# iaomw/Tracer

Measured on AMD Instinct MI355X. Metric: Mrays/s at 1920x1080x64spp, higher is better.
Workload: dtype f32

## Files before the change

### tracer_amd/csrc/dev_intersect.hpp

```cpp
#pragma once

#include "dev_prof.hpp"
#include "dev_scene.hpp"
#include "dev_vec.hpp"

namespace trcdev {

constexpr int kBlock = 64;

struct Ray {
    F3 o, d, inv;
};
TRC_DEV Ray make_ray(F3 o, F3 dir) {
    Ray r; r.o = o; r.d = normalize(dir); r.inv = rcp_cr(r.d); return r;
}
TRC_DEV F3 point_at(const Ray& r, float t) { return r.o + r.d * t; }

struct HitRec {
    float t;
    F3 p, gn, sn;
    F2 uv;
    uint32_t material;
    float PDF;
    uint32_t tag;
    F3 vol_o, vol_d;
    float vol_t;
    uint32_t vol_cube;
};
TRC_DEV void hit_init(HitRec& h) {
    h.t = 0; h.p = f3(0); h.gn = f3(0); h.sn = f3(0); h.uv.x = 0; h.uv.y = 0; h.material = 0; h.PDF = 0; h.tag = kTagNone;
    h.vol_o = f3(0); h.vol_d = f3(0); h.vol_t = 0; h.vol_cube = kTagNone;
}
TRC_DEV void check_face(HitRec& h, const Ray& ray) {
    bool f = dot(ray.d, h.gn) <= 0;
    h.sn = f ? h.gn : -h.gn;
}

struct SceneRef {
    const uint32_t* small_base;
    const uint32_t* blob;
    uint32_t off_nodes, off_spheres, off_squares, off_cubes, off_materials, off_tripos, off_triattr;
    uint32_t n_lds_nodes;
    uint32_t stack_lds;
    uint32_t stack_cap;
    uint32_t* ovf;
    uint32_t descend_min;
};
TRC_DEV float4 ld4(const uint32_t* p) { return *reinterpret_cast<const float4*>(p); }
#if defined(__HIP_DEVICE_COMPILE__)
typedef float trc_v4f __attribute__((ext_vector_type(4)));
TRC_DEV float4 ld4_global(const uint32_t* p) {
    const trc_v4f v = *(const __attribute__((address_space(1))) trc_v4f*)p;
    return make_float4(v.x, v.y, v.z, v.w);
}
TRC_DEV float4 ld4_lds(const uint32_t* p) {
    const trc_v4f v = *(const __attribute__((address_space(3))) trc_v4f*)p;
    return make_float4(v.x, v.y, v.z, v.w);
}
TRC_DEV uint32_t ld1_global(const uint32_t* p) { return *(const __attribute__((address_space(1))) uint32_t*)p; }
TRC_DEV void st1_global(uint32_t* p, uint32_t v) { *(__attribute__((address_space(1))) uint32_t*)p = v; }
#else
TRC_DEV float4 ld4_global(const uint32_t* p) { return ld4(p); }
TRC_DEV float4 ld4_lds(const uint32_t* p) { return ld4(p); }
TRC_DEV uint32_t ld1_global(const uint32_t* p) { return *p; }
TRC_DEV void st1_global(uint32_t* p, uint32_t v) { *p = v; }
#endif

template <bool ALL_LDS>
TRC_DEV void load_node(const SceneRef& S, uint32_t idx, float4& q0, float4& q1, float4& q2, float4& q3) {
    if (ALL_LDS || idx < S.n_lds_nodes) {
        const uint32_t* np = S.small_base + S.off_nodes + idx * kNodeDwords;
        q0 = ld4_lds(np); q1 = ld4_lds(np + 4); q2 = ld4_lds(np + 8); q3 = ld4_lds(np + 12);
    } else {
        const uint32_t* np = S.blob + S.off_nodes + (size_t)idx * kNodeDwords;
        q0 = ld4_global(np); q1 = ld4_global(np + 4); q2 = ld4_global(np + 8); q3 = ld4_global(np + 12);
    }
}

#ifndef TRC_WALK_TRIM
#define TRC_WALK_TRIM 1
#endif
constexpr float kRangeTMin = FLT_MIN;
static_assert(!TRC_WALK_TRIM || kRangeTMin > 0, "box_hit / box_hit_t drop `|| tmax < 0` and `tmin < 0 ? tmax : tmin`: valid for a positive lower bound only");
TRC_DEV bool box_hit(F3 mn, F3 mx, const Ray& r, float ry) {
    F3 ts = (mn - r.o) * r.inv;
    F3 te = (mx - r.o) * r.inv;
    float tmin = fmax3(fminf(ts.x, te.x), fminf(ts.y, te.y), fminf(ts.z, te.z));
    float tmax = fmin3(fmaxf(ts.x, te.x), fmaxf(ts.y, te.y), fmaxf(ts.z, te.z));
    tmin = fmaxf(tmin, kRangeTMin);
    tmax = fminf(tmax, ry);
    return !(tmax < tmin || (!TRC_WALK_TRIM && tmax < 0));
}
TRC_DEV bool box_hit_t(F3 mn, F3 mx, const Ray& r, float ry, float& t) {
    F3 ts = (mn - r.o) * r.inv;
    F3 te = (mx - r.o) * r.inv;
    float tmin = fmax3(fminf(ts.x, te.x), fminf(ts.y, te.y), fminf(ts.z, te.z));
    float tmax = fmin3(fmaxf(ts.x, te.x), fmaxf(ts.y, te.y), fmaxf(ts.z, te.z));
    tmin = fmaxf(tmin, kRangeTMin);
    tmax = fminf(tmax, ry);
    if (tmax < tmin || (!TRC_WALK_TRIM && tmax < 0)) return false;
    t = (!TRC_WALK_TRIM && tmin < 0) ? tmax : tmin;
    return true;
}

TRC_DEV float box_pad() { return 1 + 2 * ((3 * FLT_EPSILON * 0.5f) / (1 - 3 * FLT_EPSILON * 0.5f)); }

TRC_DEV bool box_hit_record(F3 mini, F3 maxi, F3 o, F3 d, float range_y, float& out_t, F3& out_gn, F3& out_p, F2& out_uv) {
    float tmin = -FLT_MAX;
    float tmax = range_y;
    uint32_t axisPick = 0;
    const F3 ddd = o - mini, bbb = o - maxi;
    const float pad = box_pad();
    const bool inside = (ddd.x > 0 && ddd.y > 0 && ddd.z > 0) && (bbb.x < 0 && bbb.y < 0 && bbb.z < 0);
#if TRC_WAVE_GUARDS
    const F3 nlo = mini - o, nhi = maxi - o;
    F3 qlo, qhi;
    {
        const GuardedDivBy bx = guarded_div_by(d.x), by = guarded_div_by(d.y), bz = guarded_div_by(d.z);
        qlo = f3(div_core(nlo.x, bx), div_core(nlo.y, by), div_core(nlo.z, bz));
        qhi = f3(div_core(nhi.x, bx), div_core(nhi.y, by), div_core(nhi.z, bz));
        const float small = fminf(fmin3(fmin3(fabsf(nlo.x), fabsf(nlo.y), fabsf(nlo.z)), fmin3(fabsf(nhi.x), fabsf(nhi.y), fabsf(nhi.z)),
                                        fmin3(fabsf(d.x), fabsf(d.y), fabsf(d.z))), 0x1p60f);
        const float large = fmax3(fmax3(fabsf(nlo.x), fabsf(nlo.y), fabsf(nlo.z)), fmax3(fabsf(nhi.x), fabsf(nhi.y), fabsf(nhi.z)),
                                  fmax3(fabsf(d.x), fabsf(d.y), fabsf(d.z)));
        if (__builtin_expect(!wave_all(small >= 0x1p-60f && large <= 0x1p60f), 0)) { qlo = nlo / d; qhi = nhi / d; }
    }
#endif
#pragma unroll
    for (uint32_t i = 0; i < 3; ++i) {
        float oi = comp(o, i), di = comp(d, i);
#if TRC_WAVE_GUARDS
        (void)oi; (void)di;
        float min_bound = comp(qlo, i);
        float max_bound = comp(qhi, i);
#else
        float min_bound = (comp(mini, i) - oi) / di;
        float max_bound = (comp(maxi, i) - oi) / di;
#endif
        float ts = fminf(max_bound, min_bound);
        float te = fmaxf(max_bound, min_bound);
        te *= pad;
        if (inside) {
            tmin = fmaxf(ts, tmin);
            if (te < tmax) { tmax = te; axisPick = i; }
        } else {
            tmax = fminf(te, tmax);
            if (ts > tmin) { tmin = ts; axisPick = i; }
        }
        if (tmax < tmin || tmax < 0) return false;
    }
    const float dpick = comp(d, axisPick);
    const float t = inside ? tmax : tmin;
    out_t = t;
    F3 gn = f3(0);
    set_comp(gn, axisPick, inside ? (dpick > 0 ? 1.0f : -1.0f) : (dpick > 0 ? -1.0f : 1.0f));
    out_gn = gn;
    F3 hitPoint = o + d * t;
    F3 p = hitPoint;
    set_comp(p, axisPick, inside ? (dpick > 0 ? comp(maxi, axisPick) : comp(mini, axisPick))
                                 : (dpick > 0 ? comp(mini, axisPick) : comp(maxi, axisPick)));
    out_p = p;
    uint32_t ax = axisPick + 1; ax = ax >= 3 ? ax - 3 : ax;
    uint32_t ay = axisPick + 2; ay = ay >= 3 ? ay - 3 : ay;
    out_uv.x = comp(hitPoint, ax);
    out_uv.y = comp(hitPoint, ay);
    return true;
}

TRC_DEV F2 sphere_uv(F3 p) {
    float phi = dm_atan2f(p.z, p.x);
    float theta = dm_asinf(p.y);
    F2 uv;
    uv.x = 1 - (phi + kPi) / (2 * kPi);
    uv.y = (theta + kPi2) / kPi;
    return uv;
}

template <bool EAGER_UV>
TRC_DEV bool sphere_hit_test(const SceneRef& S, uint32_t index, const Ray& ray, float rx, float& ry, HitRec& rec) {
    const uint32_t* sp = S.small_base + S.off_spheres + index * kSphereDwords;
    const float4 cr = ld4(sp);
    const F3 center = f3(cr.x, cr.y, cr.z);
    const float radius = cr.w;
    F3 oc = ray.o - center;
    float a = dot(ray.d, ray.d);
    float half_b = dot(oc, ray.d);
    float c = dot(oc, oc) - radius * radius;
    float discriminant = half_b * half_b - a * c;
    if (discriminant <= 0) return false;
    float root = sqrt_cr(discriminant);
    float temp = (-half_b - root) / a;
    if (!(temp < ry && temp > rx)) {
        temp = (-half_b + root) / a;
        if (!(temp < ry && temp > rx)) return false;
    }
    rec.t = temp;
    rec.p = point_at(ray, temp);
    rec.gn = div_shared(rec.p - center, radius);
    check_face(rec, ray);
    if (EAGER_UV) rec.uv = sphere_uv(rec.gn);
    rec.material = sp[4];
    ry = temp;
    return true;
}

TRC_DEV F2 square_uv(const SceneRef& S, uint32_t index, F3 p) {
    const uint32_t* sq = S.small_base + S.off_squares + index * kSquareDwords;
    const float4 rg = ld4(sq);
    const uint32_t axes = sq[6];
    const uint32_t axis_i = axes & 3u, axis_j = (axes >> 2) & 3u;
    F2 uv;
    uv.x = (comp(p, axis_i) - rg.x) / (rg.y - rg.x);
    uv.y = (comp(p, axis_j) - rg.z) / (rg.w - rg.z);
    return uv;
}
template <bool EAGER_UV = true>
TRC_DEV bool square_hit_test(const SceneRef& S, uint32_t index, const Ray& ray, float rx, float& ry, HitRec& rec) {
    const uint32_t* sq = S.small_base + S.off_squares + index * kSquareDwords;
    const float4 rg = ld4(sq);
    const float4 kx = ld4(sq + 4);
    const uint32_t axes = __float_as_uint(kx.z);
    const uint32_t axis_i = axes & 3u, axis_j = (axes >> 2) & 3u, axis_k = (axes >> 4) & 3u;
    const float value_k = kx.x;
    float t = (value_k - comp(ray.o, axis_k)) / comp(ray.d, axis_k);
    if (is_inf(t) || is_nan(t)) return false;
    if (t < rx || t > ry) return false;
    float a = comp(ray.o, axis_i) + t * comp(ray.d, axis_i);
    if (a < rg.x || a > rg.y) return false;
    float b = comp(ray.o, axis_j) + t * comp(ray.d, axis_j);
    if (b < rg.z || b > rg.w) return false;
    if (EAGER_UV) {
        rec.uv.x = (a - rg.x) / (rg.y - rg.x);
        rec.uv.y = (b - rg.z) / (rg.w - rg.z);
    }
    rec.t = t;
#if TRC_WALK_TRIM
    const bool front = comp(ray.d, axis_k) <= 0;
    const float one = front ? 1.0f : -1.0f, zero = front ? 0.0f : -0.0f;
    rec.sn = f3(axis_k == 0 ? one : zero, axis_k == 1 ? one : zero, axis_k >= 2 ? one : zero);
    rec.gn = rec.sn;
    rec.p = f3(axis_j == 0 ? b : (axis_i == 0 ? a : value_k),
               axis_j == 1 ? b : (axis_i == 1 ? a : value_k),
               axis_j >= 2 ? b : (axis_i >= 2 ? a : value_k));
#else
    F3 gn = f3(0);
    set_comp(gn, axis_k, 1.0f);
    rec.gn = gn;
    check_face(rec, ray);
    rec.gn = rec.sn;
    set_comp(rec.p, axis_k, value_k);
    set_comp(rec.p, axis_i, a);
    set_comp(rec.p, axis_j, b);
#endif
    ry = t;
    rec.PDF = kx.y;
    rec.material = __float_as_uint(kx.w);
    return true;
}

struct LightSample { F3 p, n; float areaPDF; uint32_t material; };
TRC_DEV F3 offset_ray(const F3 p, const F3 n) {
    const float origin = 1.0f / 32.0f, float_scale = 1.0f / 65536.0f, int_scale = 256.0f;
    int32_t of_x = (int32_t)(int_scale * n.x), of_y = (int32_t)(int_scale * n.y), of_z = (int32_t)(int_scale * n.z);
    float pix = __int_as_float(__float_as_int(p.x) + ((p.x < 0) ? -of_x : of_x));
    float piy = __int_as_float(__float_as_int(p.y) + ((p.y < 0) ? -of_y : of_y));
    float piz = __int_as_float(__float_as_int(p.z) + ((p.z < 0) ? -of_z : of_z));
    return f3(fabsf(p.x) < origin ? p.x + float_scale * n.x : pix,
              fabsf(p.y) < origin ? p.y + float_scale * n.y : piy,
              fabsf(p.z) < origin ? p.z + float_scale * n.z : piz);
}
TRC_DEV void square_sample(const SceneRef& S, uint32_t index, F2 u, F3 pos, LightSample& lsr) {
    const uint32_t* sq = S.small_base + S.off_squares + index * kSquareDwords;
    const float4 rg = ld4(sq);
    const float4 kx = ld4(sq + 4);
    const uint32_t axes = __float_as_uint(kx.z);
    const uint32_t axis_i = axes & 3u, axis_j = (axes >> 2) & 3u, axis_k = (axes >> 4) & 3u;
    F3 p = f3(0);
    set_comp(p, axis_k, kx.x);
    set_comp(p, axis_i, rg.x + u.x * (rg.y - rg.x));
    set_comp(p, axis_j, rg.z + u.y * (rg.w - rg.z));
    F3 n = f3(0);
    set_comp(n, axis_k, 1.0f);
    F3 w = normalize(pos - p);
    set_comp(n, axis_k, copysignf(1.0f, dot(w, n)));
    lsr.n = n;
    lsr.p = offset_ray(p, n);
    lsr.areaPDF = kx.y;
    lsr.material = __float_as_uint(kx.w);
}

template <bool STATS, bool VOL>
TRC_DEV bool cube_hit_test(const SceneRef& S, uint32_t index, const Ray& ray, float& ry, HitRec& rec, TravCounters& cnt) {
    const uint32_t* cb = S.small_base + S.off_cubes + index * kCubeDwords;
    const float4 i0 = ld4(cb), i1 = ld4(cb + 4), i2 = ld4(cb + 8);
    const F3 ic0 = f3(i0.x, i0.y, i0.z), ic1 = f3(i0.w, i1.x, i1.y), ic2 = f3(i1.z, i1.w, i2.x), ic3 = f3(i2.y, i2.z, i2.w);
    F3 origin = ((ic0 * ray.o.x + ic1 * ray.o.y) + ic2 * ray.o.z) + ic3;
    F3 direction = (ic0 * ray.d.x + ic1 * ray.d.y) + ic2 * ray.d.z;
    direction = normalize(direction);
    const F3 mini = f3(__uint_as_float(cb[33]), __uint_as_float(cb[34]), __uint_as_float(cb[35]));
    const F3 maxi = f3(__uint_as_float(cb[36]), __uint_as_float(cb[37]), __uint_as_float(cb[38]));
    float t_obj; F3 gn_obj, p_obj; F2 uv;
    if (!box_hit_record(mini, maxi, origin, direction, ry, t_obj, gn_obj, p_obj, uv)) return false;
    if (STATS) cnt.hit_cube++;
    const float4 m0 = ld4(cb + 12), m1 = ld4(cb + 16), m2 = ld4(cb + 20);
    const F3 mc0 = f3(m0.x, m0.y, m0.z), mc1 = f3(m0.w, m1.x, m1.y), mc2 = f3(m1.z, m1.w, m2.x), mc3 = f3(m2.y, m2.z, m2.w);
    F3 p = ((mc0 * p_obj.x + mc1 * p_obj.y) + mc2 * p_obj.z) + mc3;
    float t = length(ray.o - p);
    if (t >= ry) return false;
    ry = t;
    if (VOL) { rec.vol_o = origin; rec.vol_d = direction; rec.vol_t = t_obj; rec.vol_cube = index; }
    const float4 n0 = ld4(cb + 24), n1 = ld4(cb + 28);
    const F3 nc0 = f3(n0.x, n0.y, n0.z), nc1 = f3(n0.w, n1.x, n1.y), nc2 = f3(n1.z, n1.w, __uint_as_float(cb[32]));
    rec.t = t;
    rec.p = p;
    rec.gn = normalize((nc0 * gn_obj.x + nc1 * gn_obj.y) + nc2 * gn_obj.z);
    check_face(rec, ray);
    rec.uv = uv;
    rec.material = cb[39];
    return true;
}

#ifndef TRC_TRIANGLE_MATERIALS
#define TRC_TRIANGLE_MATERIALS 1
#endif
struct TriPos { float4 a, b, c; };
TRC_DEV TriPos load_tripos(const SceneRef& S, uint32_t index) {
    const uint32_t* tp = S.blob + S.off_tripos + (size_t)index * kTriPosDwords;
    TriPos t; t.a = ld4_global(tp); t.b = ld4_global(tp + 4); t.c = ld4_global(tp + 8);
    return t;
}
template <bool STATS>
TRC_DEV bool triangle_hit_test(const SceneRef& S, uint32_t index, const TriPos& pos, const Ray& ray, float rx, float& ry, HitRec& rec, TravCounters& cnt) {
    const float4 a4 = pos.a, b4 = pos.b, c4 = pos.c;
    const F3 v0 = f3(a4.x, a4.y, a4.z), v1 = f3(b4.x, b4.y, b4.z), v2 = f3(c4.x, c4.y, c4.z);
    F3 v0v1 = v1 - v0;
    F3 v0v2 = v2 - v0;
    F3 pvec = cross(ray.d, v0v2);
    float det = dot(v0v1, pvec);
    if (fabsf(det) < FLT_EPSILON) return false;
    float invDet = 1 / det;
    F3 tvec = ray.o - v0;
    float u = dot(tvec, pvec) * invDet;
    if (u < 0 || u > 1) return false;
    F3 qvec = cross(tvec, v0v1);
    float v = dot(ray.d, qvec) * invDet;
    if (v < 0 || (u + v) > 1) return false;
    float w = 1.0f - u - v;
    float t = dot(v0v2, qvec) * invDet;
    if (t > ry || t < rx) return false;
    if (STATS) cnt.hit_triangle++;
    rec.p = (u * v1 + v * v2) + w * v0;
    ry = t;
    rec.t = t;
    const uint32_t* ta = S.blob + S.off_triattr + (size_t)index * kTriAttrDwords;
    const float4 q0 = ld4(ta), q1 = ld4(ta + 4), q2 = ld4(ta + 8), q3 = ld4(ta + 12);
    const F3 n0 = f3(q0.x, q0.y, q0.z), n1 = f3(q0.w, q1.x, q1.y), n2 = f3(q1.z, q1.w, q2.x);
    rec.gn = (u * n1 + v * n2) + w * n0;
    rec.uv.x = (u * q2.w + v * q3.y) + w * q2.y;
    rec.uv.y = (u * q3.x + v * q3.z) + w * q2.z;
    check_face(rec, ray);
    rec.material = TRC_TRIANGLE_MATERIALS ? __float_as_uint(q3.w) : 19u;
    return true;
}

TRC_DEV void triangle_record(const SceneRef& S, uint32_t index, const Ray& ray, HitRec& rec) {
    const uint32_t* tp = S.blob + S.off_tripos + (size_t)index * kTriPosDwords;
    const uint32_t* ta = S.blob + S.off_triattr + (size_t)index * kTriAttrDwords;
    const float4 a4 = ld4_global(tp), b4 = ld4_global(tp + 4), c4 = ld4_global(tp + 8);
    const float4 q0 = ld4_global(ta), q1 = ld4_global(ta + 4), q2 = ld4_global(ta + 8), q3 = ld4_global(ta + 12);
    const F3 v0 = f3(a4.x, a4.y, a4.z), v1 = f3(b4.x, b4.y, b4.z), v2 = f3(c4.x, c4.y, c4.z);
    F3 v0v1 = v1 - v0;
    F3 v0v2 = v2 - v0;
    F3 pvec = cross(ray.d, v0v2);
    float det = dot(v0v1, pvec);
    float invDet = 1 / det;
    F3 tvec = ray.o - v0;
    float u = dot(tvec, pvec) * invDet;
    F3 qvec = cross(tvec, v0v1);
    float v = dot(ray.d, qvec) * invDet;
    float w = 1.0f - u - v;
    float t = dot(v0v2, qvec) * invDet;
    rec.p = (u * v1 + v * v2) + w * v0;
    rec.t = t;
    const F3 n0 = f3(q0.x, q0.y, q0.z), n1 = f3(q0.w, q1.x, q1.y), n2 = f3(q1.z, q1.w, q2.x);
    rec.gn = (u * n1 + v * n2) + w * n0;
    rec.uv.x = (u * q2.w + v * q3.y) + w * q2.y;
    rec.uv.y = (u * q3.x + v * q3.z) + w * q2.z;
    check_face(rec, ray);
    rec.material = TRC_TRIANGLE_MATERIALS ? __float_as_uint(q3.w) : 19u;
}

struct Trav {
    uint32_t tag, sp;
    float ry;
    int32_t level;
    TRC_DEV bool is_done() const { return tag == kTagNone; }
    TRC_DEV void finish() { tag = kTagNone; }
    uint32_t win_tag;
    float win_ry;
};

template <bool HYB>
TRC_DEV void stack_push(const SceneRef& S, uint32_t* stack, uint32_t& sp, uint32_t v) {
    if (!HYB || __builtin_expect(__builtin_amdgcn_ballot_w64(sp >= S.stack_lds) == 0ull, 1) || sp < S.stack_lds) stack[sp * kBlock] = v;
    else st1_global(S.ovf + (sp - S.stack_lds) * kBlock, v);
    sp++;
}
template <bool HYB>
TRC_DEV uint32_t stack_pop(const SceneRef& S, const uint32_t* stack, uint32_t& sp) {
    sp--;
    if (!HYB || __builtin_expect(__builtin_amdgcn_ballot_w64(sp >= S.stack_lds) == 0ull, 1) || sp < S.stack_lds) return stack[sp * kBlock];
    return ld1_global(S.ovf + (sp - S.stack_lds) * kBlock);
}

template <bool HYB, bool STATS>
TRC_DEV void trav_pop_or_finish(const SceneRef& S, Trav& tv, int32_t ret_start, const uint32_t* stack, const uint32_t* lvstack, TravCounters& cnt) {
    if (tv.sp == 0) {
        if (STATS) cnt.n_return += (uint32_t)(ret_start + 1);
        tv.finish();
        return;
    }
    tv.tag = stack_pop<HYB>(S, stack, tv.sp);
    if (STATS) {
        const int32_t ls = (int32_t)lvstack[tv.sp * kBlock];
        cnt.n_return += (uint32_t)(ret_start - ls + 1);
        tv.level = ls;
        if ((tv.tag >> kTagIndexBits) == kTagInterior) tv.level += 1;
    }
}

template <bool STATS>
TRC_DEV bool trav_begin(const F3 root_min, const F3 root_max, const Ray& ray, const float test_t, Trav& tv, TravCounters& cnt) {
    if (STATS) cnt.rays++;
    tv.tag = kTagNone;
    tv.sp = 0;
    tv.level = 0;
    tv.ry = test_t;
    tv.win_tag = kTagNone;
    tv.win_ry = test_t;
    const float finite_probe = fabsf(ray.o.x) + fabsf(ray.o.y) + fabsf(ray.o.z) + fabsf(ray.d.x) + fabsf(ray.d.y) + fabsf(ray.d.z);
    if (!(finite_probe < __builtin_inff())) return false;
    if (!box_hit(root_min, root_max, ray, test_t)) return false;
    tv.tag = kTagInterior << kTagIndexBits;
    return true;
}

template <bool STATS, bool EAGER_UV, bool VOL, int DEFER = 0>
TRC_DEV bool trav_test_leaf(const SceneRef& S, const Ray& ray, HitRec& rec, Trav& tv, uint32_t tag, TravCounters& cnt) {
    const float rx = kRangeTMin;
    const uint32_t type = tag >> kTagIndexBits, index = tag & kTagIndexMask;
    bool ok;
    HitRec scratch;
    HitRec& out = DEFER ? scratch : rec;
    const float ry_seen = tv.ry;
    if (type == 1u) {
        if (STATS) cnt.leaf[1]++;
        ProfScope<STATS> scope(cnt, kProfSquare);
        ok = square_hit_test<EAGER_UV>(S, index, ray, rx, tv.ry, out);
        if (DEFER && ok) rec.PDF = scratch.PDF;
    } else if (type == 0u) {
        if (STATS) cnt.leaf[0]++;
        ProfScope<STATS> scope(cnt, kProfSphere);
        ok = sphere_hit_test<EAGER_UV>(S, index, ray, rx, tv.ry, out);
    } else if (type == 2u) {
        if (STATS) cnt.leaf[2]++;
        ProfScope<STATS> scope(cnt, kProfCube);
        ok = cube_hit_test<STATS, VOL>(S, index, ray, tv.ry, DEFER == 2 ? rec : out, cnt);
        if (DEFER == 1 && VOL && ok) { rec.vol_o = scratch.vol_o; rec.vol_d = scratch.vol_d; rec.vol_t = scratch.vol_t; rec.vol_cube = scratch.vol_cube; }
    } else {
        if (STATS) cnt.leaf[3]++;
        ProfScope<STATS> scope(cnt, kProfTriangle);
        ok = triangle_hit_test<STATS>(S, index, load_tripos(S, index), ray, rx, tv.ry, out, cnt);
    }
    if (ok) {
        if (DEFER) { tv.win_tag = tag; tv.win_ry = ry_seen; }
        else rec.tag = tag;
    }
    return ok;
}
template <bool EAGER_UV, bool VOL, int DEFER>
TRC_DEV void trav_build_record(const SceneRef& S, const Ray& ray, HitRec& rec, const Trav& tv) {
    const uint32_t type = tv.win_tag >> kTagIndexBits, index = tv.win_tag & kTagIndexMask;
    TravCounters nocount;
    float ry = tv.win_ry;
    if (type == 3u) triangle_record(S, index, ray, rec);
    else if (type == 1u) { square_hit_test<EAGER_UV>(S, index, ray, kRangeTMin, ry, rec); if (!EAGER_UV) { rec.uv.x = 0; rec.uv.y = 0; } }
    else if (type == 0u) { sphere_hit_test<EAGER_UV>(S, index, ray, kRangeTMin, ry, rec); if (!EAGER_UV) { rec.uv.x = 0; rec.uv.y = 0; } }
    else if (DEFER != 2) cube_hit_test<false, VOL>(S, index, ray, ry, rec, nocount);
    rec.tag = tv.win_tag;
}

template <bool ALL_LDS, bool STATS, bool ANY, bool EAGER_UV, bool VOL = false, bool HYB = false, int DEFER = 0>
TRC_DEV void trav_iter(const SceneRef& S, const Ray& ray, HitRec& rec, const float test_t, Trav& tv,
                       uint32_t* stack, uint32_t* lvstack, TravCounters& cnt) {
#ifndef TRC_DESCEND_MIN_LDS
#define TRC_DESCEND_MIN_LDS 1
#endif
    const uint32_t kDescendMin = ALL_LDS ? (uint32_t)TRC_DESCEND_MIN_LDS : S.descend_min;
    for (;;) {
        const bool interior = (tv.tag >> kTagIndexBits) == kTagInterior;
        if (!STATS && (!ALL_LDS || TRC_DESCEND_MIN_LDS > 1)) {
            const unsigned long long m = __ballot(interior);
            if (m == 0ull) break;
            if ((uint32_t)__popcll(m) < kDescendMin && __ballot((tv.tag >> kTagIndexBits) < kTagInterior) != 0ull) break;
            if (!interior) continue;
        } else if (!interior) break;
        float4 q0, q1, q2, q3;
        load_node<ALL_LDS>(S, tv.tag & kTagIndexMask, q0, q1, q2, q3);
        if (STATS) cnt.n_descend++;
        ProfScope<STATS> scope(cnt, kProfDescend);
        float t_left = tv.ry, t_right = tv.ry;
        const bool left_test = box_hit_t(f3(q0.x, q0.y, q0.z), f3(q0.w, q1.x, q1.y), ray, tv.ry, t_left);
        const bool right_test = box_hit_t(f3(q1.z, q1.w, q2.x), f3(q2.y, q2.z, q2.w), ray, tv.ry, t_right);
        if (left_test || right_test) {
            const uint32_t tagL = __float_as_uint(q3.z), tagR = __float_as_uint(q3.w);
            const bool left_first = t_left < t_right;
            if (left_test && right_test) {
                if (STATS) lvstack[tv.sp * kBlock] = (uint32_t)tv.level;
                stack_push<HYB>(S, stack, tv.sp, left_first ? tagR : tagL);
            }
            tv.tag = left_first ? tagL : tagR;
            if (STATS && (tv.tag >> kTagIndexBits) == kTagInterior) tv.level += 1;
        } else {
            trav_pop_or_finish<HYB, STATS>(S, tv, tv.level - 1, stack, lvstack, cnt);
        }
    }
    if ((tv.tag >> kTagIndexBits) < kTagInterior) {
        trav_test_leaf<STATS, EAGER_UV, VOL, DEFER>(S, ray, rec, tv, tv.tag, cnt);
        if (ANY && tv.ry < test_t) tv.finish();
        else trav_pop_or_finish<HYB, STATS>(S, tv, tv.level, stack, lvstack, cnt);
    }
}

template <bool ALL_LDS, bool STATS, bool ANY, bool EAGER_UV, bool VOL = false, bool HYB = false, int DEFER = 0>
TRC_DEV bool scene_hit(const SceneRef& S, const F3 root_min, const F3 root_max, const Ray& ray, HitRec& rec, const float test_t,
                       uint32_t* stack, uint32_t* lvstack, TravCounters& cnt) {
    static_assert(!DEFER || (!STATS && !ANY), "the deferred record is the production closest-hit walk's");
    Trav tv;
    if (!trav_begin<STATS>(root_min, root_max, ray, test_t, tv, cnt)) return false;
    while (!tv.is_done()) trav_iter<ALL_LDS, STATS, ANY, EAGER_UV, VOL, HYB, DEFER>(S, ray, rec, test_t, tv, stack, lvstack, cnt);
    const bool hit = tv.ry < test_t;
    if (DEFER && hit) trav_build_record<EAGER_UV, VOL, DEFER>(S, ray, rec, tv);
    return hit;
}

enum : uint32_t { kOccludedNo = 0u, kOccludedYes = 1u, kOccludedAskReference = 2u };
template <bool ALL_LDS, bool VOL, bool HYB>
TRC_DEV uint32_t scene_occluded_free(const SceneRef& S, const F3 root_min, const F3 root_max, const Ray& ray, const float test_t,
                                     uint32_t* stack, const uint32_t stack_cap) {
    Trav tb;
    TravCounters nocount;
    if (!trav_begin<false>(root_min, root_max, ray, test_t, tb, nocount)) return kOccludedNo;
    constexpr uint32_t kRoot = kTagInterior << kTagIndexBits;
    uint32_t cur0 = kRoot, sp = 0;
    bool found = false, ask_reference = false;
    HitRec rec;
    hit_init(rec);
    auto is_interior = [](uint32_t tag) { return tag != kTagNone && (tag >> kTagIndexBits) == kTagInterior; };
    auto is_leaf = [](uint32_t tag) { return tag != kTagNone && (tag >> kTagIndexBits) != kTagInterior; };
    bool restarted = false;
    auto give = [&](uint32_t tag) {
        if (restarted) return;
        if (cur0 == kTagNone) cur0 = tag;
        else if (sp < stack_cap) stack_push<HYB>(S, stack, sp, tag);
        else { restarted = true; sp = 0; cur0 = kTagNone; found = true; ask_reference = true; }
    };
#ifndef TRC_OCCL_DESCEND_MIN
#define TRC_OCCL_DESCEND_MIN 1
#endif
    constexpr int kDescendMin = ALL_LDS ? TRC_DESCEND_MIN_LDS : TRC_OCCL_DESCEND_MIN;
    for (;;) {
        for (;;) {
            const bool i0 = is_interior(cur0);
            const unsigned long long m = __ballot(i0);
            if (m == 0ull) break;
            if (__popcll(m) < kDescendMin && __ballot(is_leaf(cur0)) != 0ull) break;
            if (!i0) continue;
            float4 a0, a1, a2, a3;
            const uint32_t t0 = cur0;
            restarted = false;
            load_node<ALL_LDS>(S, t0 & kTagIndexMask, a0, a1, a2, a3);
            cur0 = kTagNone;
            auto expand = [&](const float4& q0, const float4& q1, const float4& q2, const float4& q3) {
                float t_left = test_t, t_right = test_t;
                const bool l = box_hit_t(f3(q0.x, q0.y, q0.z), f3(q0.w, q1.x, q1.y), ray, test_t, t_left);
                const bool r = box_hit_t(f3(q1.z, q1.w, q2.x), f3(q2.y, q2.z, q2.w), ray, test_t, t_right);
                const uint32_t tagL = __float_as_uint(q3.z), tagR = __float_as_uint(q3.w);
                if (l && r) { give(tagL); give(tagR); }
                else if (l || r) give(t_left < t_right ? tagL : tagR);
            };
            expand(a0, a1, a2, a3);
            if (restarted) continue;
            if (cur0 == kTagNone && sp > 0u) cur0 = stack_pop<HYB>(S, stack, sp);
        }
        if (!found && is_leaf(cur0)) {
            Trav tv;
            tv.ry = test_t;
            if (trav_test_leaf<false, false, VOL>(S, ray, rec, tv, cur0, nocount)) {
                if (tv.ry < test_t) found = true;
                else if (!(tv.ry == test_t)) { found = true; ask_reference = true; }
            }
            cur0 = kTagNone;
        }
        if (found) { cur0 = kTagNone; sp = 0; }
        if (cur0 == kTagNone && sp > 0u) cur0 = stack_pop<HYB>(S, stack, sp);
        if (__ballot(cur0 != kTagNone) == 0ull) break;
    }
    return ask_reference ? kOccludedAskReference : (found ? kOccludedYes : kOccludedNo);
}
template <bool ALL_LDS, bool VOL, bool HYB>
TRC_DEV bool scene_occluded(const SceneRef& S, const F3 root_min, const F3 root_max, const Ray& ray, const float test_t,
                            uint32_t* stack, const uint32_t stack_cap) {
    const uint32_t r = scene_occluded_free<ALL_LDS, VOL, HYB>(S, root_min, root_max, ray, test_t, stack, stack_cap);
    if (r != kOccludedAskReference) return r == kOccludedYes;
    HitRec rec;
    hit_init(rec);
    TravCounters nocount;
    return scene_hit<ALL_LDS, false, true, false, VOL, HYB>(S, root_min, root_max, ray, rec, test_t, stack, nullptr, nocount);
}

}
```

Baseline: 15100.

## Walk BVH by raw LDS byte addresses and trim box-hit record selection

In the all-LDS, non-stats, non-hybrid traversal, the stack pointer and node indices become raw LDS byte addresses. Node loads compute the address with one shift-add from the tag, and push/pop index the stack directly, removing per-step index multiplies and masking. The pop-or-finish is rewritten as a branchless load guarded by a base compare. Separately, the box-hit-record path precomputes near/far slabs and picks the normal, point and uv with selects instead of dynamic component indexing. The address trick relies on the tag's type bits being shifted out and on a fixed 64-byte node size.

```diff
diff --git a/tracer_amd/csrc/dev_intersect.hpp b/tracer_amd/csrc/dev_intersect.hpp
--- a/tracer_amd/csrc/dev_intersect.hpp
+++ b/tracer_amd/csrc/dev_intersect.hpp
@@ -59,11 +59,22 @@
 }
 TRC_DEV uint32_t ld1_global(const uint32_t* p) { return *(const __attribute__((address_space(1))) uint32_t*)p; }
 TRC_DEV void st1_global(uint32_t* p, uint32_t v) { *(__attribute__((address_space(1))) uint32_t*)p = v; }
+TRC_DEV uint32_t lds_addr(const uint32_t* p) { return (uint32_t)(uintptr_t)(const __attribute__((address_space(3))) uint32_t*)p; }
+TRC_DEV float4 ld4_lds_at(uint32_t a) {
+    const trc_v4f v = *(const __attribute__((address_space(3))) trc_v4f*)(uintptr_t)a;
+    return make_float4(v.x, v.y, v.z, v.w);
+}
+TRC_DEV uint32_t ld1_lds_at(uint32_t a) { return *(const __attribute__((address_space(3))) uint32_t*)(uintptr_t)a; }
+TRC_DEV void st1_lds_at(uint32_t a, uint32_t v) { *(__attribute__((address_space(3))) uint32_t*)(uintptr_t)a = v; }
 #else
 TRC_DEV float4 ld4_global(const uint32_t* p) { return ld4(p); }
 TRC_DEV float4 ld4_lds(const uint32_t* p) { return ld4(p); }
 TRC_DEV uint32_t ld1_global(const uint32_t* p) { return *p; }
 TRC_DEV void st1_global(uint32_t* p, uint32_t v) { *p = v; }
+TRC_DEV uint32_t lds_addr(const uint32_t*) { return 0u; }
+TRC_DEV float4 ld4_lds_at(uint32_t) { return make_float4(0, 0, 0, 0); }
+TRC_DEV uint32_t ld1_lds_at(uint32_t) { return 0u; }
+TRC_DEV void st1_lds_at(uint32_t, uint32_t) {}
 #endif
 
 template <bool ALL_LDS>
@@ -115,6 +126,9 @@
 #if TRC_WAVE_GUARDS
     const F3 nlo = mini - o, nhi = maxi - o;
     F3 qlo, qhi;
+#if TRC_WALK_TRIM
+    F3 near, far;
+#endif
     {
         const GuardedDivBy bx = guarded_div_by(d.x), by = guarded_div_by(d.y), bz = guarded_div_by(d.z);
         qlo = f3(div_core(nlo.x, bx), div_core(nlo.y, by), div_core(nlo.z, bz));
@@ -123,7 +137,17 @@
                                         fmin3(fabsf(d.x), fabsf(d.y), fabsf(d.z))), 0x1p60f);
         const float large = fmax3(fmax3(fabsf(nlo.x), fabsf(nlo.y), fabsf(nlo.z)), fmax3(fabsf(nhi.x), fabsf(nhi.y), fabsf(nhi.z)),
                                   fmax3(fabsf(d.x), fabsf(d.y), fabsf(d.z)));
-        if (__builtin_expect(!wave_all(small >= 0x1p-60f && large <= 0x1p60f), 0)) { qlo = nlo / d; qhi = nhi / d; }
+#if TRC_WALK_TRIM
+        near = f3(fminf(qhi.x, qlo.x), fminf(qhi.y, qlo.y), fminf(qhi.z, qlo.z));
+        far = f3(fmaxf(qhi.x, qlo.x), fmaxf(qhi.y, qlo.y), fmaxf(qhi.z, qlo.z));
+#endif
+        if (__builtin_expect(!wave_all(small >= 0x1p-60f && large <= 0x1p60f), 0)) {
+            qlo = nlo / d; qhi = nhi / d;
+#if TRC_WALK_TRIM
+            near = f3(fminf(qhi.x, qlo.x), fminf(qhi.y, qlo.y), fminf(qhi.z, qlo.z));
+            far = f3(fmaxf(qhi.x, qlo.x), fmaxf(qhi.y, qlo.y), fmaxf(qhi.z, qlo.z));
+#endif
+        }
     }
 #endif
 #pragma unroll
@@ -137,8 +161,14 @@
         float min_bound = (comp(mini, i) - oi) / di;
         float max_bound = (comp(maxi, i) - oi) / di;
 #endif
+#if TRC_WAVE_GUARDS && TRC_WALK_TRIM
+        (void)min_bound; (void)max_bound;
+        float ts = comp(near, i);
+        float te = comp(far, i);
+#else
         float ts = fminf(max_bound, min_bound);
         float te = fmaxf(max_bound, min_bound);
+#endif
         te *= pad;
         if (inside) {
             tmin = fmaxf(ts, tmin);
@@ -149,9 +179,21 @@
         }
         if (tmax < tmin || tmax < 0) return false;
     }
-    const float dpick = comp(d, axisPick);
     const float t = inside ? tmax : tmin;
     out_t = t;
+#if TRC_WALK_TRIM
+    const bool a0 = axisPick == 0, a1 = axisPick == 1, a2 = !a0 && !a1;
+    const float dpick = a0 ? d.x : (a1 ? d.y : d.z);
+    const bool far_face = inside == (dpick > 0);
+    const float one = far_face ? 1.0f : -1.0f;
+    out_gn = f3(a0 ? one : 0.0f, a1 ? one : 0.0f, a2 ? one : 0.0f);
+    const F3 hitPoint = o + d * t;
+    out_p = f3(a0 ? (far_face ? maxi.x : mini.x) : hitPoint.x, a1 ? (far_face ? maxi.y : mini.y) : hitPoint.y,
+               a2 ? (far_face ? maxi.z : mini.z) : hitPoint.z);
+    out_uv.x = a0 ? hitPoint.y : (a1 ? hitPoint.z : hitPoint.x);
+    out_uv.y = a0 ? hitPoint.z : (a1 ? hitPoint.x : hitPoint.y);
+#else
+    const float dpick = comp(d, axisPick);
     F3 gn = f3(0);
     set_comp(gn, axisPick, inside ? (dpick > 0 ? 1.0f : -1.0f) : (dpick > 0 ? -1.0f : 1.0f));
     out_gn = gn;
@@ -164,6 +206,7 @@
     uint32_t ay = axisPick + 2; ay = ay >= 3 ? ay - 3 : ay;
     out_uv.x = comp(hitPoint, ax);
     out_uv.y = comp(hitPoint, ay);
+#endif
     return true;
 }
 
@@ -413,6 +456,24 @@
     return ld1_global(S.ovf + (sp - S.stack_lds) * kBlock);
 }
 
+constexpr bool walk_by_address(bool all_lds, bool stats, bool hyb) { return TRC_WALK_TRIM && all_lds && !stats && !hyb; }
+constexpr uint32_t kStackRowBytes = kBlock * 4u;
+static_assert(kLdsSceneBytes / (kNodeDwords * 4u) <= (1u << (32u - 6u)) && kNodeDwords * 4u == 64u, "node_addr shifts the tag's type bits out");
+TRC_DEV uint32_t node_addr(uint32_t nodes, uint32_t tag) {
+    uint32_t a = (tag << 6) + nodes;
+#if defined(__HIP_DEVICE_COMPILE__)
+    asm("" : "+v"(a));
+#endif
+    return a;
+}
+
+TRC_DEV void trav_pop_or_finish_addr(Trav& tv, const uint32_t stack_base) {
+    const bool some = tv.sp != stack_base;
+    tv.sp -= kStackRowBytes;
+    uint32_t tag = kTagNone;
+    if (some) tag = ld1_lds_at(tv.sp);
+    tv.tag = tag;
+}
 template <bool HYB, bool STATS>
 TRC_DEV void trav_pop_or_finish(const SceneRef& S, Trav& tv, int32_t ret_start, const uint32_t* stack, const uint32_t* lvstack, TravCounters& cnt) {
     if (tv.sp == 0) {
@@ -497,6 +558,9 @@
 #define TRC_DESCEND_MIN_LDS 1
 #endif
     const uint32_t kDescendMin = ALL_LDS ? (uint32_t)TRC_DESCEND_MIN_LDS : S.descend_min;
+    constexpr bool ADDR = walk_by_address(ALL_LDS, STATS, HYB);
+    const uint32_t stack_base = ADDR ? lds_addr(stack) : 0u;
+    const uint32_t nodes = ADDR ? lds_addr(S.small_base + S.off_nodes) : 0u;
     for (;;) {
         const bool interior = (tv.tag >> kTagIndexBits) == kTagInterior;
         if (!STATS && (!ALL_LDS || TRC_DESCEND_MIN_LDS > 1)) {
@@ -506,6 +570,10 @@
             if (!interior) continue;
         } else if (!interior) break;
         float4 q0, q1, q2, q3;
+        if constexpr (ADDR) {
+            const uint32_t np = node_addr(nodes, tv.tag);
+            q0 = ld4_lds_at(np); q1 = ld4_lds_at(np + 16u); q2 = ld4_lds_at(np + 32u); q3 = ld4_lds_at(np + 48u);
+        } else
         load_node<ALL_LDS>(S, tv.tag & kTagIndexMask, q0, q1, q2, q3);
         if (STATS) cnt.n_descend++;
         ProfScope<STATS> scope(cnt, kProfDescend);
@@ -517,10 +585,14 @@
             const bool left_first = t_left < t_right;
             if (left_test && right_test) {
                 if (STATS) lvstack[tv.sp * kBlock] = (uint32_t)tv.level;
+                if constexpr (ADDR) { st1_lds_at(tv.sp, left_first ? tagR : tagL); tv.sp += kStackRowBytes; }
+                else
                 stack_push<HYB>(S, stack, tv.sp, left_first ? tagR : tagL);
             }
             tv.tag = left_first ? tagL : tagR;
             if (STATS && (tv.tag >> kTagIndexBits) == kTagInterior) tv.level += 1;
+        } else if constexpr (ADDR) {
+            trav_pop_or_finish_addr(tv, stack_base);
         } else {
             trav_pop_or_finish<HYB, STATS>(S, tv, tv.level - 1, stack, lvstack, cnt);
         }
@@ -528,6 +600,7 @@
     if ((tv.tag >> kTagIndexBits) < kTagInterior) {
         trav_test_leaf<STATS, EAGER_UV, VOL, DEFER>(S, ray, rec, tv, tv.tag, cnt);
         if (ANY && tv.ry < test_t) tv.finish();
+        else if constexpr (ADDR) trav_pop_or_finish_addr(tv, stack_base);
         else trav_pop_or_finish<HYB, STATS>(S, tv, tv.level, stack, lvstack, cnt);
     }
 }
@@ -538,6 +611,7 @@
     static_assert(!DEFER || (!STATS && !ANY), "the deferred record is the production closest-hit walk's");
     Trav tv;
     if (!trav_begin<STATS>(root_min, root_max, ray, test_t, tv, cnt)) return false;
+    if constexpr (walk_by_address(ALL_LDS, STATS, HYB)) tv.sp = lds_addr(stack);
     while (!tv.is_done()) trav_iter<ALL_LDS, STATS, ANY, EAGER_UV, VOL, HYB, DEFER>(S, ray, rec, test_t, tv, stack, lvstack, cnt);
     const bool hit = tv.ry < test_t;
     if (DEFER && hit) trav_build_record<EAGER_UV, VOL, DEFER>(S, ray, rec, tv);
```

Result: no change. 15160 (median of 6 runs) (+0.4%).
